# RobotControlLab/nimblephysics

Hardware: AMD Instinct MI355X
Metric: differentiable timesteps/sec (fwd+bwd), 1024-env Atlas w/ contact (higher is better)
Workload: dtype f64; 1 GPU; Atlas 33-DoF (atlas_v3_box_colliders) + ground, foot contact; worlds_per_gpu=1024, dofs=33, global_batch=1024, parallelism=independent worlds x1, launcher=single process

## Files before the change

### nimblephysics_amd/csrc/capi.cpp

```cpp
#include <hip/hip_runtime.h>

#include <cmath>
#include <cstdlib>
#include <cstdio>
#include <cstring>
#include <string>
#include <vector>

#include "model.h"
#include "pool_sizes.h"

static thread_local std::string g_err;

static int fail(int code, const std::string& msg) {
  g_err = msg;
  return code;
}

#define HIP_TRY(expr)                                                        \
  do {                                                                       \
    hipError_t _e = (expr);                                                  \
    if (_e != hipSuccess) return fail(NIMBLE_ERR_HIP, std::string(#expr) + ": " + hipGetErrorString(_e)); \
  } while (0)

// ... 171 lines not shown
    dofCount += m.ndof[b];
    if (m.jtype[b] == NIMBLE_JOINT_FREE || m.jtype[b] == NIMBLE_JOINT_BALL) {
      if (m.numFree >= 8) { delete w; return fail(NIMBLE_ERR_UNSUPPORTED, "more than 8 free / ball joints"); }
      m.freeBody[m.numFree++] = b;
    }
  }
  if (dofCount != m.n) { delete w; return fail(NIMBLE_ERR_INVALID, "dof count mismatch"); }
  {
    int k = 0;
    for (int lev = 0; lev <= m.maxDepth; lev++) {
      m.levelStart[lev] = k;
      for (int b = 0; b < m.nb; b++)
        if (m.depth[b] == lev) m.levelBodies[k++] = b;
    }
    m.levelStart[m.maxDepth + 1] = k;
    k = 0;
    for (int p = 0; p < m.nb; p++) {
      m.childStart[p] = k;
      for (int b = 0; b < m.nb; b++)
        if (m.parent[b] == p) m.childList[k++] = b;
    }
    m.childStart[m.nb] = k;
    k = 0;
    for (int lev = m.maxDepth; lev >= 1; lev--)
      for (int b = 0; b < m.nb; b++)
        if (m.depth[b] == lev && m.parent[b] >= 0) { m.accEdge[k][0] = m.parent[b]; m.accEdge[k][1] = b; k++; }
    m.numAcc = k;
  }
  for (int b = 0; b < m.nb; b++) {
    bool hasDof = false;
    for (int a = b; a >= 0; a = m.parent[a]) if (m.ndof[a] > 0) { hasDof = true; break; }
    m.reactive[b] = (d->skeleton_mobile[b] && hasDof) ? 1 : 0;
  }
  for (int i = 0; i < m.n; i++) {
    m.damping[i] = d->damping[i]; m.spring[i] = d->spring[i]; m.rest[i] = d->rest_position[i];
    m.posLo[i] = d->pos_lower[i]; m.posHi[i] = d->pos_upper[i];
    m.velLo[i] = d->vel_lower[i]; m.velHi[i] = d->vel_upper[i];
    m.forceLo[i] = d->force_lower[i]; m.forceHi[i] = d->force_upper[i];
  }
  for (int sIdx = 0; sIdx < m.ns; sIdx++) {
    m.shapeBody[sIdx] = d->shape_body[sIdx];
    m.shapeType[sIdx] = d->shape_type[sIdx];
    for (int i = 0; i < 3; i++) m.shapeSize[sIdx][i] = d->shape_size[3 * sIdx + i];
    std::memcpy(m.shapeT[sIdx], d->shape_T + 12 * sIdx, 12 * sizeof(double));
  }
  m.helperPrio = 0;
  if (const char* e = getenv("NIMBLE_AMD_HELPER_PRIO")) m.helperPrio = atoi(e) & 3;
  m.postSplit = 1;
  if (const char* e = getenv("NIMBLE_AMD_POST_SPLIT")) m.postSplit = atoi(e) != 0;
  m.pinvMfma = 1;
  if (const char* e = getenv("NIMBLE_AMD_PINV_MFMA")) m.pinvMfma = atoi(e) != 0 ? 1 : 0;
  m.bwdMFuse = 1;
  if (const char* e = getenv("NIMBLE_AMD_BWD_MFUSE")) m.bwdMFuse = atoi(e) != 0 ? 1 : 0;
  m.bwdSolve2 = 1;
  if (const char* e = getenv("NIMBLE_AMD_BWD_SOLVE2")) m.bwdSolve2 = atoi(e) != 0 ? 1 : 0;
  m.guardSites = 0;
  m.guardStride = 1;
  m.guardOffset = 0;
  if (const char* e = getenv("NIMBLE_AMD_GUARD_TEST")) {
    int sites = 0, stride = 1, offset = 0;
    if (sscanf(e, "%d:%d:%d", &sites, &stride, &offset) >= 1 && stride > 0 && offset >= 0 && offset < stride) {
      m.guardSites = sites;
      m.guardStride = stride;
      m.guardOffset = offset;
    }
  }
  m.numPairs = 0;
  m.pairChunk = 0;
  for (int i = 0; i < m.ns; i++)
    for (int j = i + 1; j < m.ns; j++) {
      int bi = m.shapeBody[i], bj = m.shapeBody[j];
      if (bi == bj) continue;
      int si = m.skel[bi], sj = m.skel[bj];
      if (!d->skeleton_mobile[bi] && !d->skeleton_mobile[bj]) continue;
      if (si == sj) continue;
      m.pairA[m.numPairs] = i;
      m.pairB[m.numPairs] = j;
      m.numPairs++;
    }
  m.pairChunk = m.numPairs < CT_PAIR_CHUNK_HOST ? m.numPairs : CT_PAIR_CHUNK_HOST;
  {
    std::vector<double> mv;
    m.hasMesh = 0;
    for (int sIdx = 0; sIdx < m.ns; sIdx++) {
      m.meshFirst[sIdx] = 0; m.meshCount[sIdx] = 0; m.meshRadius[sIdx] = 0.0;
      if (m.shapeType[sIdx] != NIMBLE_SHAPE_MESH) continue;
      if (d->mesh_vertices == nullptr || d->shape_mesh_count == nullptr || d->shape_mesh_count[sIdx] <= 0) {
        delete w;
        return fail(NIMBLE_ERR_INVALID, "mesh shape without vertices");
      }
      const int f = d->shape_mesh_first[sIdx], c = d->shape_mesh_count[sIdx];
      if (f < 0 || f + c > d->num_mesh_vertices) { delete w; return fail(NIMBLE_ERR_INVALID, "mesh vertex range"); }
      m.meshFirst[sIdx] = (int)(mv.size() / 3);
      double r2 = 0.0;
      for (int k = 0; k < c; k++) {
        const double* v = d->mesh_vertices + 3 * (size_t)(f + k);
        double q = 0.0;
        for (int i = 0; i < 3; i++) q += (v[i] * m.shapeSize[sIdx][i]) * (v[i] * m.shapeSize[sIdx][i]);
        if (q > r2) r2 = q;
        if (d->mesh_vertex_candidate != nullptr && d->mesh_vertex_candidate[f + k] == 0) continue;
        mv.insert(mv.end(), v, v + 3);
      }
      m.meshCount[sIdx] = (int)(mv.size() / 3) - m.meshFirst[sIdx];
      m.meshRadius[sIdx] = std::sqrt(r2);
      if (m.meshCount[sIdx] <= 0) {
        delete w;
// ... 43 lines not shown
    if (w->meshDev) (void)hipFree(w->meshDev);
    delete w;
    return fail(NIMBLE_ERR_UNSUPPORTED, "model too large for LDS");
  }
  w->bwd = makeLayout(m, true, bwdRows);
  w->fwdWide = w->fwd;
  w->wideLds = (size_t)w->fwd.total * sizeof(double);
  {
    const int mc = 3 * maxContacts < NIMBLE_MAX_SOLVED_LCP ? 3 * maxContacts : NIMBLE_MAX_SOLVED_LCP;
    const int wsd = 4 * mc + (mc + 1) / 2 + 3;
    int need = mc * mc + wsd + 65 * mc + 512;
    const int needL = mc * (mc | 1) + 2 * mc;
    if (needL > need) need = needL;
    const int room = (int)(160 * 1024 / sizeof(double)) - w->fwd.pool;
    const char* ev = getenv("NIMBLE_AMD_WIDE_STAGE");
    const bool on = !(ev && atoi(ev) == 0);
    if (m.numPairs > 0 && mc > 64 && on && room > 0) {
      const int cap = need < room ? need : room;
      w->fwdWide.stage = w->fwd.pool;
      w->fwdWide.stageCap = cap;
      const size_t end = (size_t)(w->fwd.pool + cap) * sizeof(double);
      if (end > w->wideLds) w->wideLds = end;
    }
    w->fwdDeferRows = w->deferRows;
    if (w->fwdWide.stageCap > 0 && fwdPoolDoublesHost(64, m.n) <= w->fwdWide.stageCap && fwdRows < w->fwdDeferRows) {
      const char* ef = getenv("NIMBLE_AMD_WIDE_POOL");
      if (!(ef && atoi(ef) == 0)) w->fwdDeferRows = fwdRows;
    }
    if (const char* e = getenv("NIMBLE_AMD_FWD_DEFER_ROWS")) {
      const int d = atoi(e);
      if (d >= 0 && d < w->fwdDeferRows && w->fwdWide.stageCap > 0) w->fwdDeferRows = d;
    }
    if (getenv("NIMBLE_AMD_VERBOSE"))
      fprintf(stderr, "nimble_amd: wide forward LDS %zu B (stage %d doubles of %d for %d rows), forward defers > %d rows\n",
              w->wideLds, w->fwdWide.stageCap, need, mc, w->fwdDeferRows);
  }
  if (getenv("NIMBLE_AMD_VERBOSE"))
    fprintf(stderr, "nimble_amd: LDS forward %d B (pool rows %d, early rows at %d), backward %d B (pool rows %d), max rows %d\n",
            w->fwd.total * 8, fwdRows, w->fwd.early, w->bwd.total * 8, bwdRows, mcap);
  const int poolRows = fwdRows < bwdRows ? fwdRows : bwdRows;
  w->poolRows = poolRows;
  w->maxRows = mcap;
  if (m.numPairs > 0) {
    int ws = 0;
    if (mcap > poolRows || mcap > w->fwdDeferRows) {
      const int a = fwdPoolDoublesHost(mcap, m.n), b = bwdPoolDoublesHost(mcap, m.n);
      ws = a > b ? a : b;
    }
    w->snapDoubles = snapWorkspaceOffsetHost(m.n) + ws;
  } else {
    w->snapDoubles = 8;
  }
  if (m.numPairs > 0 && bwdPoolDoublesHost(mcap, m.n) > w->bwd.poolCap) w->jacWsDoubles = bwdPoolDoublesHost(mcap, m.n);
  w->fwd.snDyn = w->bwd.snDyn = w->fwdWide.snDyn = w->snapDoubles;
  w->snapDoubles += dynCacheDoubles(m.n, m.nb);
  m.lay[0] = w->fwd;
  m.lay[1] = w->bwd;
  hipError_t e = hipMalloc(&w->dev, sizeof(ModelDev));
  if (e != hipSuccess) {
    if (w->meshDev) (void)hipFree(w->meshDev);
    delete w;
    return fail(NIMBLE_ERR_HIP, std::string("hipMalloc: ") + hipGetErrorString(e));
  }
  e = hipMemcpy(w->dev, &m, sizeof(ModelDev), hipMemcpyHostToDevice);
  if (e != hipSuccess) {
    (void)hipFree(w->dev);
    if (w->meshDev) (void)hipFree(w->meshDev);
    delete w;
    return fail(NIMBLE_ERR_HIP, std::string("hipMemcpy: ") + hipGetErrorString(e));
  }
  {
    std::vector<double> bi((size_t)m.nb * 10);
    for (int b = 0; b < m.nb; b++) {
      double* r = bi.data() + 10 * b;
      r[0] = m.mass[b];
      for (int i = 0; i < 3; i++) r[1 + i] = m.com[b][i];
      r[4] = m.Ic[b][0]; r[5] = m.Ic[b][4]; r[6] = m.Ic[b][8];
      r[7] = m.Ic[b][1]; r[8] = m.Ic[b][2]; r[9] = m.Ic[b][5];
    }
    e = hipMalloc(&w->inertiaDev, bi.size() * sizeof(double));
    if (e == hipSuccess) e = hipMemcpy(w->inertiaDev, bi.data(), bi.size() * sizeof(double), hipMemcpyHostToDevice);
    if (e != hipSuccess) {
      if (w->inertiaDev) (void)hipFree(w->inertiaDev);
      (void)hipFree(w->dev);
      if (w->meshDev) (void)hipFree(w->meshDev);
      delete w;
      return fail(NIMBLE_ERR_HIP, std::string("body parameters: ") + hipGetErrorString(e));
    }
  }
  *out = w;
  return NIMBLE_OK;
}

int nimble_world_destroy(nimble_world_t w) {
  if (!w) return NIMBLE_OK;
  if (w->dev) (void)hipFree(w->dev);
  if (w->inertiaDev) (void)hipFree(w->inertiaDev);
  if (w->meshDev) (void)hipFree(w->meshDev);
  delete w;
  return NIMBLE_OK;
}

int64_t nimble_snapshot_doubles(nimble_world_t w) { return w ? w->snapDoubles : -1; }
int64_t nimble_lcp_cache_doubles(nimble_world_t w) { return w ? w->cacheDoubles : -1; }
int32_t nimble_num_collision_pairs(nimble_world_t w) { return w ? w->host.numPairs : -1; }

// ... 407 lines not shown
```

### nimblephysics_amd/csrc/contact.cuh

```cuda
#pragma once
#include "model.h"
#include "spatial.cuh"
#include "pool_sizes.h"
#include "capsule.cuh"
#include "mesh.cuh"
#include "inertia.cuh"

#define CT_FACE_VERTEX 1
#define CT_VERTEX_FACE 2
#define CT_EDGE_EDGE 3
#include "stamp.cuh"

#define CM_CLAMPING (-1)
#define CM_NOT_CLAMPING (-2)


__device__ int deviceBoxBox(const double* p1, const double* R1, const double* A, const double* p2,
                            const double* R2, const double* B, double clipDepth, int b1, int b2, double* out) {
#pragma clang fp contract(off)
  const double fudge = 1.05;
  double p[3] = {p2[0] - p1[0], p2[1] - p1[1], p2[2] - p1[2]};
  double pp[3];
  for (int i = 0; i < 3; i++) pp[i] = R1[i] * p[0] + R1[3 + i] * p[1] + R1[6 + i] * p[2];
  double Rm[9], Qm[9];
// ... 2513 lines not shown
  helperWait(ct, [](int v) { return v != HS_POSTDONE; }, GW_HELPER_IDLE);
}

template <bool kWide>
__device__ void helperWave(const ModelDev& md, double* s, const Layout& L, int lane, double* g_stamp, double* hbmPool,
                           double* snap) {
  (void)g_stamp;
  s = lds<true>(s);
  double* ct = s + L.ct;
  int st = helperWait(ct, [](int v) { return v == HS_TASK || v == HS_SKIP || (!kWide && v == HS_POST); },
                      GW_HELPER_TASK);
  if (st < 0) return;
  if (!kWide && st == HS_POST) {
    helperPostShare(md, s, L, ct, snap, lane);
    return;
  }
  if (st == HS_TASK) {
    const int prio = md.helperPrio;
    if (prio == 1) __builtin_amdgcn_s_setprio(1);
    else if (prio == 2) __builtin_amdgcn_s_setprio(2);
    else if (prio == 3) __builtin_amdgcn_s_setprio(3);
    const int m = uni((int)ct[H_M]);
    const int mode = uni(helperFlags(ct)[1]);
    FwdPool P;
    if (kWide && mode == HB_WIDE) {
      carveFwd(gbl(hbmPool), m, md.n, P);
      lds_double* Ldz = (lds_double*)(s + L.pool);
      helperTask<false, 2, true>(md, ct, P, m, lane, Ldz, Ldz + dantzigLDoubles(m, true), sp<false>(P.M2), g_stamp);
    } else {
      carveFwd(s + L.pool, m, md.n, P);
      helperTask<true, 1>(md, ct, P, m, lane, sp<true>(P.M2), sp<true>(P.xh2), sp<true>(P.M2), g_stamp);
    }
  }
  __builtin_amdgcn_s_setprio(0);
  helperPost(ct, HS_DONE, lane);
  st = helperWait(ct, [](int v) { return v != HS_DONE; }, GW_HELPER_IDLE);
  if (!kWide && st == HS_POST) helperPostShare(md, s, L, ct, snap, lane);
}

__device__ __forceinline__ void helperRetire(double* s, const Layout& L, int lane) {
  double* ct = lds<true>(s) + L.ct;
  if (helperState(ct) == HS_IDLE) helperPost(ct, HS_SKIP, lane);
  helperWait(ct, [](int v) { return v == HS_DONE || v == HS_POSTDONE; }, GW_RETIRE);
  helperPost(ct, HS_IDLE, lane);
}

enum { NV_DELTA = 0, NV_NU, NV_SIGMA, NV_KAPPA, NV_MA1, NV_MARHO, NV_MA2, NV_MAPI, NV_YF, NV_W, NV_W2, NV_MU, NV_T0 };


struct BwdPool {
  double *gRows, *TAB, *NV;
  double *fc, *bc, *bounce, *u, *lam, *beta, *xq, *rho, *piv, *zeta, *r1;
  int* rowOf;
};

__device__ inline void carveBwd(double* base, int m, int n, BwdPool& P) {
  double* p = base;
  P.gRows = p; p += n * m;
  P.TAB = p; p += 12 * m;
  P.NV = p; p += NV_COLS * n;
  P.fc = p; p += m;
  P.bc = p; p += m;
  P.bounce = p; p += m;
  P.u = p; p += m;
  P.lam = p; p += m;
  P.beta = p; p += m;
  P.xq = p; p += m;
  P.rho = p; p += m;
  P.piv = p; p += m;
  P.zeta = p; p += m;
  P.r1 = p; p += m;
  P.rowOf = reinterpret_cast<int*>(p);
}

__device__ __forceinline__ unsigned long long ancestorDofMask(const ModelDev& md, unsigned long long bodies, int lane) {
  const bool in = lane < md.n && ((bodies >> md.dofBody[lane < md.n ? lane : 0]) & 1ull);
  return __ballot(in);
}

__device__ inline void bodyTwist(const ModelDev& md, const double* Sw, int b, const double* g, int ld, double* T) {
  for (int i = 0; i < 6; i++) T[i] = 0.0;
  if (b < 0) return;
  const unsigned long long a = md.anc[b];
#pragma unroll 4
  for (int r = 0; r < md.n; r++) {
    const double gr = ((a >> md.dofBody[r]) & 1ull) ? g[r * ld] : 0.0;
    for (int i = 0; i < 6; i++) T[i] = fma(Sw[6 * r + i], gr, T[i]);
  }
}

__device__ void tangentBasisGradient(const double* nrm, const double* g, double* T0, double* T1) {
  const double ez[3] = {0, 0, 1}, ex[3] = {1, 0, 0}, ey[3] = {0, 1, 0};
  const double* cr = ez;
  double t[3];
  cross3(cr, nrm, t);
  if (dot3(t, t) < 1e-12) {
    cr = ex; cross3(cr, nrm, t);
    if (dot3(t, t) < 1e-12) {
      cr = ey; cross3(cr, nrm, t);
      if (dot3(t, t) < 1e-12) { cr = ez; cross3(cr, nrm, t); }
    }
  }
  const double tn = sqrt(dot3(t, t));
  for (int i = 0; i < 3; i++) t[i] /= tn;
  double gc[3];
  cross3(cr, g, gc);
  for (int i = 0; i < 3; i++) gc[i] /= tn;
  double gt[3];
  if (fabs(tn - 1.0) > 1e-6) {
    const double dd = dot3(gc, t);
    for (int i = 0; i < 3; i++) gt[i] = gc[i] - dd * t[i];
  } else {
// ... 157 lines not shown
      rMap[q] = (int)rr[RR_MAP];
      if (rMap[q] == CM_CLAMPING) rC[q] = (int)rr[RR_CIDX];
      else if (rMap[q] >= 0) { rC[q] = (int)rows[rMap[q] * SN_ROWREC + RR_CIDX]; rE[q] = rr[RR_EVAL]; }
    }
  }
  {
    const int i = lane;
    const bool live = i < n;
    const double* nv = P.NV + (live ? i : 0) * NV_COLS;
    const double w = nv[NV_W], sg = nv[NV_SIGMA], ka = nv[NV_KAPPA], ma1 = nv[NV_MA1], mar = nv[NV_MARHO];
    const double ma2 = nv[NV_MA2], map = nv[NV_MAPI], vf = sn[SN_VF + (live ? i : 0)];
    for (int j = 0; j < m; j++) {
      const int mp = rdliR(rMap, j);
      const int c = rdliR(rC, j);
      const double e = rdlR(rE, j);
      double g = 0.0;
      if (mp == CM_CLAMPING) {
        g = P.fc[c] * w - P.beta[c] * vf - P.lam[c] * sg - P.xq[c] * ka;
        if (imp) g += P.rho[c] * ma1 + P.r1[c] * mar + P.piv[c] * ma2 + P.zeta[c] * map;
      } else if (mp >= 0) {
        double inner = P.fc[c] * w - P.xq[c] * ka;
        if (imp) inner += P.rho[c] * ma1 + P.piv[c] * ma2;
        g = e * inner;
      }
      if (live) P.gRows[j * n + i] = g;
    }
  }
  WSYNC();
  {
    auto bodyOf = [&](int t) {
      if (t >= 2 * m) return -1;
      const double* rec = sn + SN_CONTACTS + (int)rows[(t >> 1) * SN_ROWREC + RR_CONTACT] * CREC;
      return (int)rec[8 + (t & 1)];
    };
    unsigned long long anAll = 0ull;
    for (int t = lane; t < 2 * m; t += WAVE) {
      const int body = bodyOf(t);
      if (body >= 0) anAll |= md.anc[body];
    }
    unsigned lo = (unsigned)anAll, hi = (unsigned)(anAll >> 32);
    for (int o = 32; o >= 1; o >>= 1) {
      lo |= __shfl_xor(lo, o);
      hi |= __shfl_xor(hi, o);
    }
    const unsigned long long all = ((unsigned long long)uni((int)hi) << 32) | (unsigned)uni((int)lo);
    const unsigned long long dmAll = ancestorDofMask(md, all, lane);
    for (int t0 = 0; t0 < 2 * m; t0 += WAVE) {
      const int t = t0 + lane;
      const int body = bodyOf(t);
      const unsigned long long an = body >= 0 ? md.anc[body] : 0ull;
      unsigned long long dm = dmAll;
      double T[6] = {0, 0, 0, 0, 0, 0};
      const double* g = P.gRows + (t < 2 * m ? (t >> 1) : 0) * n;
      while (dm) {
        const int r = __ffsll((long long)dm) - 1;
        dm &= dm - 1ull;
        const double gr = ((an >> md.dofBody[r]) & 1ull) ? g[r] : 0.0;
        for (int i = 0; i < 6; i++) T[i] = fma(s[L.Sw + 6 * r + i], gr, T[i]);
      }
      if (t < 2 * m)
        for (int i = 0; i < 6; i++) P.TAB[(t >> 1) * 12 + (t & 1) * 6 + i] = T[i];
    }
  }
  WSYNC();
  STAMP(38);
  return imp;
}

__device__ double sphereRowTerm(const ModelDev& md, const double* s, const Layout& L, const BwdPool& P, int j,
                                const double* rec, const double* rr, const double* Z, int bk) {
  const int A = (int)rec[8], B = (int)rec[9], typ = (int)rec[7], type = typ & 15;
  const bool pa = (md.anc[A] >> bk) & 1ull, pb = (md.anc[B] >> bk) & 1ull;
  if (pa == pb) return 0.0;
  const bool sphereToBox = type == CT_SPHERE_BOX ? pa : pb;
  const int mask = (typ >> 4) & 7, shape = typ >> 8;
  const double* p = rec;
  const double* nrm = rec + 3;
  const double* c = rec + 10;
  const double wv[3] = {Z[0], Z[1], Z[2]};
  const bool rotates = sqrt(Z[0] * Z[0] + Z[1] * Z[1] + Z[2] * Z[2]) > 1e-6;
  auto gwt = [&](const double* x, double* o) {
    if (rotates) { cross3(wv, x, o); for (int i = 0; i < 3; i++) o[i] += Z[3 + i]; }
    else { for (int i = 0; i < 3; i++) o[i] = Z[3 + i]; }
  };
  auto lockProject = [&](double* x) {
    if (!mask) return;
    const double* Tw = s + L.Tw + 12 * md.shapeBody[shape];
    const double* Ts = md.shapeT[shape];
    for (int f = 0; f < 3; f++) {
      if (!((mask >> f) & 1)) continue;
      double fn[3];
      for (int r = 0; r < 3; r++) fn[r] = Tw[4 * r] * Ts[f] + Tw[4 * r + 1] * Ts[4 + f] + Tw[4 * r + 2] * Ts[8 + f];
      const double d0 = dot3(fn, x);
      for (int i = 0; i < 3; i++) x[i] -= fn[i] * d0;
    }
  };
  double sg[3], dp[3], dn[3];
  gwt(c, sg);
  double dist2 = 0.0;
  for (int i = 0; i < 3; i++) dist2 += (c[i] - p[i]) * (c[i] - p[i]);
  const double norm = sqrt(dist2);
  const double inv = norm > 1e-5 ? 1.0 / norm : 1.0;
  if (sphereToBox) {
    for (int i = 0; i < 3; i++) dp[i] = sg[i];
    lockProject(dp);
    for (int i = 0; i < 3; i++) {
      const double cpg = dp[i] * inv, spg = sg[i] * inv;
      dn[i] = type == CT_BOX_SPHERE ? cpg - spg : spg - cpg;
    }
  } else {
    double neg[3], pg[3];
// ... 355 lines not shown
  const int n = md.n, nb = md.nb;
  const double* rows = sn + SN_ROWS;
  double* omega = ws;
  double* Pc = ws + 6 * n;
  double* UV = Pc + 6 * nb;
  const int k = lane;
  const int bk = k < n ? md.dofBody[k] : 0;
  const int lam = k < n ? md.parent[bk] : -1;
  double acc = 0.0;
  unsigned long long done = 0ull;
  unsigned lo = 0u, hi = 0u;
  if (k < n) {
    if (bk < 32) lo = 1u << bk;
    else hi = 1u << (bk - 32);
  }
  for (int o = 32; o >= 1; o >>= 1) {
    lo |= __shfl_xor(lo, o);
    hi |= __shfl_xor(hi, o);
  }
  const unsigned long long dofBodies = ((unsigned long long)uni((int)hi) << 32) | (unsigned)uni((int)lo);
  int rMap[R], rA[R], rB[R], rTyp[R], rDir[R], rCon[R];
  double rp[3][R], rd[3][R], rn[3][R];
  unsigned long long liveRows[R];
#pragma unroll
  for (int q = 0; q < R; q++) {
    const int j = rowAt(q, lane);
    rMap[q] = CM_NOT_CLAMPING; rA[q] = 0; rB[q] = 0; rTyp[q] = 0; rDir[q] = 0; rCon[q] = 0;
    for (int i = 0; i < 3; i++) { rp[i][q] = 0.0; rd[i][q] = 0.0; rn[i][q] = 0.0; }
    if (j < m) {
      const double* rr = rows + j * SN_ROWREC;
      rMap[q] = (int)rr[RR_MAP];
      rDir[q] = (int)rr[RR_DIR];
      rCon[q] = (int)rr[RR_CONTACT];
      const double* rec = sn + SN_CONTACTS + rCon[q] * CREC;
      rA[q] = (int)rec[8]; rB[q] = (int)rec[9]; rTyp[q] = (int)rec[7];
      for (int i = 0; i < 3; i++) { rp[i][q] = rec[i]; rn[i][q] = rec[3 + i]; rd[i][q] = rr[RR_D + i]; }
    }
    liveRows[q] = __ballot(j < m && rMap[q] != CM_NOT_CLAMPING);
  }
  for (int j0 = 0; j0 < m; j0++) {
    if (!bitR(liveRows, j0)) continue;
    for (int side = 0; side < 2; side++) {
      const int c = side ? rdliR(rB, j0) : rdliR(rA, j0);
      if ((done >> c) & 1ull) continue;
      done |= 1ull << c;
      if (!(md.anc[c] & dofBodies)) continue;
      TACC_BEGIN(tO);
      double om[6] = {0, 0, 0, 0, 0, 0};
      unsigned long long rowsC[R];
#pragma unroll
      for (int q = 0; q < R; q++) rowsC[q] = __ballot(((liveRows[q] >> lane) & 1ull) && (rA[q] == c || rB[q] == c));
#pragma unroll
      for (int q = 0; q < R; q++)
      for (unsigned long long bits = rowsC[q]; bits; bits &= bits - 1ull) {
        const int j = 64 * q + __ffsll((long long)bits) - 1;
        const double sg = rdliR(rA, j) == c ? 1.0 : -1.0;
        double p[3], d[3];
        for (int i = 0; i < 3; i++) { p[i] = rdlR(rp[i], j); d[i] = rdlR(rd[i], j); }
        double wr[6];
        cross3(p, d, wr);
        wr[3] = d[0]; wr[4] = d[1]; wr[5] = d[2];
        if (lane < n) {
          const double gr = sg * P.gRows[j * n + lane];
#pragma unroll
          for (int i = 0; i < 6; i++) om[i] = fma(gr, wr[i], om[i]);
        }
      }
      {
        double uvl[6] = {0, 0, 0, 0, 0, 0};
#pragma unroll
        for (int q = 0; q < R; q++) {
          const int type = rTyp[q] & 15;
          const bool vertexSide = ((rowsC[q] >> lane) & 1ull) && ((type == CT_VERTEX_FACE && rA[q] == c) ||
                                                                   (type == CT_FACE_VERTEX && rB[q] == c));
          if (vertexSide) {
            const int j = rowAt(q, lane);
            double tw[3], dxt[3], pxd[3], dj[3], pj[3];
            for (int i = 0; i < 3; i++) {
              tw[i] = P.TAB[j * 12 + i] - P.TAB[j * 12 + 6 + i];
              dj[i] = rd[i][q];
              pj[i] = rp[i][q];
            }
            cross3(dj, tw, dxt);
            cross3(pj, dxt, pxd);
            for (int i = 0; i < 3; i++) { uvl[i] += dxt[i]; uvl[3 + i] += pxd[i]; }
          }
        }
        double uvs[6];
        for (int i = 0; i < 6; i++) uvs[i] = waveSum(uvl[i]);
        if (lane == 0)
          for (int i = 0; i < 6; i++) UV[i] = uvs[i];
      }
      if (lane < n)
        for (int i = 0; i < 6; i++) omega[lane * 6 + i] = om[i];
      WSYNC();
      TACC_END(82, tO);
      TACC_BEGIN(tP);
      if (lane < n) {
        double t[6];
        crf(s + L.Sw + 6 * lane, omega + 6 * lane, t);
        for (int i = 0; i < 6; i++) omega[lane * 6 + i] = t[i];
      }
      WSYNC();
      {
        unsigned long long dm = ancestorDofMask(md, md.anc[c], lane);
        if (lane < nb) {
          double pb[6] = {0, 0, 0, 0, 0, 0};
          const unsigned long long an = md.anc[lane];
          while (dm) {
            const int r = __ffsll((long long)dm) - 1;
            dm &= dm - 1ull;
            const double w = ((an >> md.dofBody[r]) & 1ull) ? 1.0 : 0.0;
#pragma unroll
            for (int i = 0; i < 6; i++) pb[i] = fma(w, omega[6 * r + i], pb[i]);
          }
          for (int i = 0; i < 6; i++) Pc[lane * 6 + i] = pb[i];
        }
      }
// ... 200 lines not shown
```

### nimblephysics_amd/csrc/model.h

```cpp
#pragma once
#include <stdint.h>

#include "../../include/nimble_amd.h"

inline int jointDofs(int jt) {
  switch (jt) {
    case NIMBLE_JOINT_WELD: return 0;
    case NIMBLE_JOINT_REVOLUTE: case NIMBLE_JOINT_PRISMATIC: return 1;
    case NIMBLE_JOINT_BALL: case NIMBLE_JOINT_TRANSLATIONAL: return 3;
    case NIMBLE_JOINT_FREE: return 6;
    default: return -1;
  }
}

#define NB_MAX NIMBLE_MAX_BODIES
#define ND_MAX NIMBLE_MAX_DOFS
#define NS_MAX NIMBLE_MAX_SHAPES

struct Layout {
  int q, v, tau, Tw, Sw, V, A, IC, F, M, rhs, x, scratch;
  int adj, Wt, w, gp, gv;
  int ct, v1, pool, poolCap, dinv;
  int snDyn;
  int cscr;
  int stage, stageCap;
  int early;
  int total;
};

struct ModelDev {
  int nb, n, ns, maxDepth;
  int numFree;
  int freeBody[8];
  double dt, g[3], clipDepth, fallbackCfm;
  int penCorr, parallelPosVel;
  int parent[NB_MAX], jtype[NB_MAX], dof0[NB_MAX], ndof[NB_MAX], depth[NB_MAX];
  int skel[NB_MAX], reactive[NB_MAX];
  unsigned long long anc[NB_MAX];
  int levelStart[NB_MAX + 1], levelBodies[NB_MAX];
  int childStart[NB_MAX + 1], childList[NB_MAX];
  int numAcc;
  int accEdge[NB_MAX][2];
  double Tpj[NB_MAX][12];
  double Tcj[NB_MAX][12];
  double TcjInv[NB_MAX][12];
  double axis[NB_MAX][3];
  double mass[NB_MAX], com[NB_MAX][3], Ic[NB_MAX][9];
  double friction[NB_MAX], restitution[NB_MAX];
  int dofBody[ND_MAX];
  double damping[ND_MAX], spring[ND_MAX], rest[ND_MAX];
  double posLo[ND_MAX], posHi[ND_MAX], velLo[ND_MAX], velHi[ND_MAX], forceLo[ND_MAX], forceHi[ND_MAX];
  int shapeBody[NS_MAX], shapeType[NS_MAX];
  double shapeSize[NS_MAX][3];
  double shapeT[NS_MAX][12];
  const double* meshVerts;
  int meshFirst[NS_MAX], meshCount[NS_MAX];
  double meshRadius[NS_MAX];
  int hasMesh;
  int helperPrio;
  int postSplit;
  int pinvMfma;
  int bwdMFuse;
  int bwdSolve2;
  int guardSites, guardStride, guardOffset;
  int maxContacts;
  int numPairs, pairChunk;
  int pairA[NS_MAX * (NS_MAX - 1) / 2], pairB[NS_MAX * (NS_MAX - 1) / 2];
  Layout lay[2];
};
```

### nimblephysics_amd/csrc/pool_sizes.h

```cpp
#pragma once
#include <hip/hip_runtime.h>

#include "../../include/nimble_amd.h"

#define CREC 13
#define EDGE_REC 12
#define PBREC (CREC + EDGE_REC)

#define CT_CONTACTS 32
#define CT_MAX_DROPPED 64
#define DROP_REC 3
#define CT_PAIR_CHUNK 16
#define CT_PAIR_CHUNK_HOST CT_PAIR_CHUNK
#define DEFER_BUCKETS 4
#define MESH_PAIR_RECS 64
#define MESH_PAIR_SCRATCH (16 * 64)
__host__ __device__ inline int ctDoubles(int maxContacts) { return CT_CONTACTS + maxContacts * CREC; }
__host__ __device__ inline int pairBufRecs(int pairChunk, bool mesh) {
  return mesh ? (MESH_PAIR_RECS > 8 * pairChunk ? MESH_PAIR_RECS : 8 * pairChunk) : 8 * pairChunk;
}
__host__ __device__ inline int collideScratchDoubles(int pairChunk, bool mesh) {
  return CT_MAX_DROPPED * DROP_REC + pairBufRecs(pairChunk, mesh) * PBREC + (mesh ? MESH_PAIR_SCRATCH : 0);
}

#define SN_NCON 0
#define SN_M 1
#define SN_NC 2
#define SN_NU 3
#define SN_CFM 4
#define SN_STATUS 5
#define SN_SC 6
#define SN_IGN 7
#define SN_IMP 8
#define SN_PIVOTS 9
#define SN_SWEEPS 10
#define SN_SOLVER_FLOPS 11
#define SN_DEFER 12
#define SN_DEFERCNT 14
#define SN_CONTACTS 16
#define SN_ROWS (SN_CONTACTS + NIMBLE_MAX_CONTACTS * CREC)
#define SN_ROWREC 12
#define SN_FC (SN_ROWS + NIMBLE_MAX_LCP * SN_ROWREC)
#define SN_VF (SN_FC + NIMBLE_MAX_LCP)
#define SN_MAXL NIMBLE_MAX_LCP
static_assert(SN_PIVOTS == NIMBLE_SNAPSHOT_PIVOTS && SN_SWEEPS == NIMBLE_SNAPSHOT_SWEEPS &&
                  SN_SOLVER_FLOPS == NIMBLE_SNAPSHOT_SOLVER_FLOPS && SN_DEFERCNT + 2 <= SN_CONTACTS,
              "include/nimble_amd.h snapshot offsets");
static_assert(SN_FC == NIMBLE_SNAPSHOT_FC && SN_NC == NIMBLE_SNAPSHOT_NUM_CLAMPING,
              "include/nimble_amd.h snapshot offsets");
__host__ __device__ inline int snAlign8(int x) { return ((x + 7) / 8) * 8; }
__host__ __device__ inline int snYf(int n) { return SN_VF + n; }
__host__ __device__ inline int snAc(int n) { return snAlign8(snYf(n) + n); }
__host__ __device__ inline int snAcubE(int n) { return snAc(n) + n * SN_MAXL; }
__host__ __device__ inline int snPT(int n) { return snAcubE(n) + n * SN_MAXL; }
__host__ __device__ inline int snQ(int n) { return snPT(n) + SN_MAXL * SN_MAXL; }
__host__ __device__ inline int snEdge(int n) { return snQ(n) + SN_MAXL * SN_MAXL; }
#ifdef NIMBLE_STAGE_TIMING
#define SN_DEBUG_TAIL 128
#else
#define SN_DEBUG_TAIL 0
#endif
__host__ __device__ inline int snStamps(int n) { return snAlign8(snEdge(n) + NIMBLE_MAX_CONTACTS * EDGE_REC); }
__host__ __device__ inline int snapWorkspaceOffset(int n) { return snStamps(n) + SN_DEBUG_TAIL; }

#define NV_COLS 16
__host__ __device__ inline int fwdPoolDoubles(int m, int n) { return n * m + 3 * m * m + 33 * m + 2 * n + 72; }
__host__ __device__ inline int bwdPoolDoubles(int m, int n) { return n * m + 24 * m + NV_COLS * n + 64; }

__host__ __device__ inline int fwdPoolRowsDoubles(int m, int n) { return n * m + 10 * m; }

#define fwdPoolDoublesHost fwdPoolDoubles
#define bwdPoolDoublesHost bwdPoolDoubles
#define snapWorkspaceOffsetHost snapWorkspaceOffset

__host__ __device__ inline int dynCacheDoubles(int n, int nb) {
  return 12 * nb + 6 * n + 6 * nb + n * (n + 1) / 2 + n + n;
}
```

### nimblephysics_amd/csrc/timestep.hip

```cpp
#include <hip/hip_runtime.h>

#include "model.h"
#include "spatial.cuh"
#include "wave.cuh"
#include "stamp.cuh"
#include "chol_wave.cuh"
#include "inertia.cuh"
#include "wrench.cuh"

#define WAVE 64

#if defined(NIMBLE_PER_WORLD_KERNELS)
#define NIMBLE_SHARED_MODEL_INSTANCES 0
#define NIMBLE_PER_WORLD_INSTANCES 1
#define NIMBLE_EXT_WRENCH_INSTANCES 0
#elif defined(NIMBLE_EXT_WRENCH_KERNELS)
#define NIMBLE_SHARED_MODEL_INSTANCES 0
#define NIMBLE_PER_WORLD_INSTANCES 0
#define NIMBLE_EXT_WRENCH_INSTANCES 1
#elif defined(__HIP__)
#define NIMBLE_SHARED_MODEL_INSTANCES 1
#define NIMBLE_PER_WORLD_INSTANCES 0
#define NIMBLE_EXT_WRENCH_INSTANCES 0
#else
// ... 609 lines not shown
  const ModelDev& md = *mdp;
  const Layout& L = md.lay[1];
  const int lane = threadIdx.x;
  const int n = md.n;
  const double dt = md.dt;
  const long long items = (long long)batch * rows;
  for (long long item = blockIdx.x; item < items; item += gridDim.x) {
    const int env = rows == 1 ? (int)item : (int)(item / rows);
    const int unitRow = rows == 1 ? -1 : (int)(item - (long long)env * rows);
    if (md.numPairs > 0) {
      const int mEnv = uni((int)snapshot[(size_t)env * snapDoubles + SN_M]);
      if ((mEnv > deferRows) != (R > 1)) continue;
    }
#ifdef NIMBLE_STAGE_TIMING
    double* g_stamp = md.numPairs > 0 ? snapshot + (size_t)env * snapDoubles + snStamps(n) : nullptr;
#endif
    STAMP(20);
    if (fcMode && (md.numPairs == 0 || unitRow >= uni((int)snapshot[(size_t)env * snapDoubles + SN_NC]))) {
      for (int i = lane; i < 2 * n; i += WAVE) gradState[(size_t)item * 2 * n + i] = 0.0;
      for (int i = lane; i < n; i += WAVE) gradForces[(size_t)item * n + i] = 0.0;
      if constexpr (kExt)
        if (gradWrench != nullptr)
          for (int i = lane; i < 6 * md.nb; i += WAVE) gradWrench[(size_t)item * 6 * md.nb + i] = 0.0;
      continue;
    }
    loadState(md, s, L, lane, state + (size_t)env * 2 * n, forces + (size_t)env * n);
    if (fcMode) {
      for (int i = lane; i < n; i += WAVE) { s[L.gp + i] = 0.0; s[L.gv + i] = 0.0; }
    } else if (unitRow < 0) {
      const double* gN = gradNext + (size_t)env * 2 * n;
      for (int i = lane; i < n; i += WAVE) {
        s[L.gp + i] = gN[i];
        s[L.gv + i] = gN[n + i];
      }
    } else {
      for (int i = lane; i < n; i += WAVE) {
        s[L.gp + i] = i == unitRow ? 1.0 : 0.0;
        s[L.gv + i] = n + i == unitRow ? 1.0 : 0.0;
      }
    }
    const double* bi = !kPW ? nullptr
                       : kExt ? bodyInertia + (size_t)env * inertiaStride
                              : bodyInertia + (size_t)env * md.nb * 10;
    double* sn = snapshot + (size_t)env * snapDoubles;
    double* hbmWs = ws != nullptr ? ws + (size_t)blockIdx.x * wsDoubles : sn + snapWorkspaceOffset(n);
    dynCacheCopy(md, s, L, sn + L.snDyn, false, lane);
    STAMP(21);
    const int nc = md.numPairs > 0 ? uni((int)sn[SN_NC]) : 0;
    const int m = md.numPairs > 0 ? uni((int)sn[SN_M]) : 0;
    double* x = s + L.x;
    double* w = s + L.w;
    BwdPool P;
    int imp = 0;
    if (nc > 0) {
      const int need = bwdPoolDoubles(m, n);
      carveBwd(need <= L.poolCap ? s + L.pool : hbmWs, m, n, P);
      imp = contactBackwardPrep<R>(md, s, L, lane, sn, P, m, nc, s + L.ct, fcMode ? unitRow : -1);
    } else {
      for (int i = lane; i < n; i += WAVE) {
        const double qi = s[L.q + i], vi = s[L.v + i];
        const double springF = md.spring[i] * (qi - md.rest[i] + dt * vi);
        const double dampF = md.damping[i] * vi;
        x[i] = dt * (s[L.tau + i] - s[L.rhs + i] - dampF - springF);
        w[i] = s[L.gv + i];
      }
      WSYNC();
      if (md.bwdSolve2) {
        double xw[2] = {lane < n ? x[lane] : 0.0, lane < n ? w[lane] : 0.0};
        cholSolveReg<2>(s + L.M, s + L.dinv, xw, n, lane);
        WSYNC();
        if (lane < n) { x[lane] = xw[0]; w[lane] = xw[1]; }
        WSYNC();
      } else {
        cholSolve(s + L.M, s + L.dinv, x, n, lane);
        cholSolve(s + L.M, s + L.dinv, w, n, lane);
      }
      for (int i = lane; i < n; i += WAVE) x[i] /= dt;
      WSYNC();
    }
    STAMP(22);
    accelerations(md, s, L, lane, x, s + L.adj);
    if constexpr (kExt) {
      adjointVectors<kPW, true>(md, s, L, lane, bi, bodyWrench + (size_t)env * md.nb * 6, wrenchFrame);
      if (gradWrench != nullptr && lane < md.nb) {
        const int b = lane;
        double Wd[6], gw[6];
        for (int i = 0; i < 6; i++) Wd[i] = dt * s[L.Wt + 6 * b + i];
        twistInWrenchFrame(Wd, wrenchFrame, s + L.Tw + 12 * b, gw);
        for (int i = 0; i < 6; i++) gradWrench[((size_t)item * md.nb + b) * 6 + i] = gw[i];
      }
    } else {
      adjointVectors<kPW>(md, s, L, lane, bi);
    }
    STAMP(23);

    double gq = 0.0, gvOut = 0.0, gt = 0.0;
    double Z[6] = {0, 0, 0, 0, 0, 0};
    const int k = lane;
    if (k < n) {
      const int b = md.dofBody[k];
      const int lam = md.parent[b];
      const double ag[6] = {0, 0, 0, md.g[0], md.g[1], md.g[2]};
      double Vl[6], ul[6];
      for (int i = 0; i < 6; i++) {
        Vl[i] = lam >= 0 ? s[L.V + 6 * lam + i] : 0.0;
        ul[i] = (lam >= 0 ? s[L.A + 6 * lam + i] : 0.0) - ag[i];
      }
      const double* Sk = s + L.Sw + 6 * k;
      if (md.jtype[b] == NIMBLE_JOINT_FREE || md.jtype[b] == NIMBLE_JOINT_BALL) {
// ... 6 lines not shown
        } else {
          double Rm[9];
          expMapRot(th, Rm);
          for (int r = 0; r < 3; r++) xi[3 + r] = Rm[(c - 3) * 3 + r];
        }
        double TwC[12];
        tmul(s + L.Tw + 12 * b, md.Tcj[b], TwC);
        adT(TwC, xi, Z);
      } else {
        for (int i = 0; i < 6; i++) Z[i] = Sk[i];
      }
      const double* a = s + L.adj + 42 * b;
      double t[6], r[6], acc6[6];
      crf(Vl, a + 6, t);
      for (int i = 0; i < 6; i++) r[i] = a[12 + i] + t[i] + a[24 + i] - a[30 + i];
      crf(Vl, r, t);
      crf(ul, a + 6, r);
      for (int i = 0; i < 6; i++) acc6[i] = -a[i] - r[i] + t[i] + a[18 + i] + a[36 + i];
      const double accQ = dot6(Z, acc6);
      double vs[6];
      for (int i = 0; i < 6; i++) vs[i] = Vl[i] + s[L.V + 6 * b + i];
      crf(vs, a + 6, t);
      for (int i = 0; i < 6; i++) acc6[i] = -t[i] - a[12 + i] - a[24 + i] + a[30 + i];
      const double accV = dot6(Sk, acc6);
      const double wk = w[k];
      gq = -dt * accQ - dt * md.spring[k] * wk;
      gvOut = s[L.gv + k] - dt * accV - dt * md.damping[k] * wk - dt * dt * md.spring[k] * wk;
      gt = dt * wk;
      if (nc > 0) gvOut -= P.NV[k * NV_COLS + NV_MU];
      if (md.jtype[b] != NIMBLE_JOINT_FREE && md.jtype[b] != NIMBLE_JOINT_BALL) {
        gq += s[L.gp + k];
        gvOut += dt * s[L.gp + k];
      }
    }
    WSYNC();
    STAMP(24);
    if (nc > 0) {
      double* buf = s + L.adj;
      TACC_BEGIN(tG);
#ifdef NIMBLE_STAGE_TIMING
      const double gterm = contactGTermsAll<R>(md, s, L, sn, P, m, Z, buf, lane, g_stamp);
#else
      const double gterm = contactGTermsAll<R>(md, s, L, sn, P, m, Z, buf, lane);
#endif
      WSYNC();
      TACC_END(80, tG);
      TACC_BEGIN(tM);
      bool mfuse = false;
      double* wI = buf + 24 * md.nb;
      const double* NVf = P.NV;
      int ldNV = NV_COLS;
      if (md.bwdMFuse) {
        const int wId = (13 * md.nb + 1) & ~1;
        const bool onChip = bwdPoolDoubles(m, n) <= L.poolCap;
        int idle = onChip ? 0 : L.poolCap;
        double* free = s + L.pool;
        if (n * (n + 1) / 2 >= wId) { mfuse = true; wI = s + L.M; }
        else if (onChip && (n + 12) * m >= wId) { mfuse = true; wI = P.gRows; }
        else if (idle >= wId) { mfuse = true; wI = free; free += wId; idle -= wId; }
        if (mfuse) {
          if (idle >= 8 * n) {
            double* stage = free;
            if (lane < n)
              for (int c = 0; c < 8; c++) stage[lane * 8 + c] = P.NV[lane * NV_COLS + c];
            NVf = stage;
            ldNV = 8;
          }
        }
      }
#ifdef NIMBLE_STAGE_TIMING
      const double mterm = mFieldsTerm<kPW>(md, s, L, NVf, ldNV, buf, wI, mfuse, lane, k, Z, -dt, (double)imp, g_stamp, bi);
#else
      const double mterm = mFieldsTerm<kPW>(md, s, L, NVf, ldNV, buf, wI, mfuse, lane, k, Z, -dt, (double)imp, bi);
#endif
      TACC_END(81, tM);
      if (k < n) {
        gq += gterm;
        gq += mterm;
      }
      WSYNC();
    }
    STAMP(25);
    if (gradMasses != nullptr) {
      if (lane < md.nb) {
        const int b = lane;
        const double* Tw = s + L.Tw + 12 * b;
        const double m = kPW ? bi[10 * b] : md.mass[b];
        const double* cb = kPW ? bi + 10 * b + 1 : md.com[b];
        double cw[3];
        for (int r = 0; r < 3; r++)
          cw[r] = Tw[r * 4] * cb[0] + Tw[r * 4 + 1] * cb[1] + Tw[r * 4 + 2] * cb[2] + Tw[r * 4 + 3];
        auto comVel = [&](const double* y, double* u) {
          double cx[3];
          cross3(cw, y, cx);
          for (int i = 0; i < 3; i++) u[i] = y[3 + i] - cx[i];
        };
        auto bodyAng = [&](const double* y, double* wb) {
          for (int i = 0; i < 3; i++) wb[i] = Tw[i] * y[0] + Tw[4 + i] * y[1] + Tw[8 + i] * y[2];
        };
        auto pairTerms = [&](const double* x, const double* y, double coef, double* out) {
          double ux[3], uy[3];
          comVel(x, ux);
          comVel(y, uy);
          out[0] += coef * (ux[0] * uy[0] + ux[1] * uy[1] + ux[2] * uy[2]);
          if (massParams < 10) return;
          for (int k = 0; k < 3; k++) {
            const double rk[3] = {Tw[k], Tw[4 + k], Tw[8 + k]};
            double a[3], c[3];
            cross3(x, rk, a);
            cross3(y, rk, c);
            out[1 + k] += coef * m * (a[0] * uy[0] + a[1] * uy[1] + a[2] * uy[2] + ux[0] * c[0] + ux[1] * c[1] + ux[2] * c[2]);
          }
          double bx[3], by[3];
          bodyAng(x, bx);
// ... 183 lines not shown
```

Measured before the change: 3.154 million timesteps/s.

## Split backward contact pool between LDS and HBM with batched off-chip row loads

Adds tiered placement for the backward contact pool. When the whole pool does not fit in LDS, only the large gRows block (or gRows plus TAB) goes to HBM workspace and the vector arrays stay on-chip. Before, everything spilled to HBM. For off-chip gRows, the TAB build loop and the omega accumulation loop batch eight row loads before the FMA work, so the global-memory latency overlaps. A host check rejects models whose tiered placement does not fit, and the NV staging path is now limited to the full-HBM tier. This adds code size and register pressure, and the gain only shows when contact rows exceed LDS capacity.

```diff
diff --git a/nimblephysics_amd/csrc/capi.cpp b/nimblephysics_amd/csrc/capi.cpp
--- a/nimblephysics_amd/csrc/capi.cpp
+++ b/nimblephysics_amd/csrc/capi.cpp
@@ -247,6 +247,8 @@
   if (const char* e = getenv("NIMBLE_AMD_PINV_MFMA")) m.pinvMfma = atoi(e) != 0 ? 1 : 0;
   m.bwdMFuse = 1;
   if (const char* e = getenv("NIMBLE_AMD_BWD_MFUSE")) m.bwdMFuse = atoi(e) != 0 ? 1 : 0;
+  m.bwdPoolSplit = 1;
+  if (const char* e = getenv("NIMBLE_AMD_BWD_POOL_SPLIT")) m.bwdPoolSplit = atoi(e) != 0 ? 1 : 0;
   m.bwdSolve2 = 1;
   if (const char* e = getenv("NIMBLE_AMD_BWD_SOLVE2")) m.bwdSolve2 = atoi(e) != 0 ? 1 : 0;
   m.guardSites = 0;
@@ -396,6 +398,18 @@
     w->snapDoubles = 8;
   }
   if (m.numPairs > 0 && bwdPoolDoublesHost(mcap, m.n) > w->bwd.poolCap) w->jacWsDoubles = bwdPoolDoublesHost(mcap, m.n);
+  if (m.numPairs > 0) {
+    const int wsSnap = w->snapDoubles - snapWorkspaceOffsetHost(m.n);
+    for (int r = 0; r <= mcap; r++) {
+      const int tier = bwdPoolTier(r, m.n, w->bwd.poolCap, m.bwdPoolSplit);
+      const int off = bwdPoolHbmDoubles(tier, r, m.n);
+      if (bwdPoolChipDoubles(tier, r, m.n) > w->bwd.poolCap || off > wsSnap || (off > 0 && off > w->jacWsDoubles)) {
+        if (w->meshDev) (void)hipFree(w->meshDev);
+        delete w;
+        return fail(NIMBLE_ERR_UNSUPPORTED, "backward pool placement does not fit for " + std::to_string(r) + " rows");
+      }
+    }
+  }
   w->fwd.snDyn = w->bwd.snDyn = w->fwdWide.snDyn = w->snapDoubles;
   w->snapDoubles += dynCacheDoubles(m.n, m.nb);
   m.lay[0] = w->fwd;
diff --git a/nimblephysics_amd/csrc/contact.cuh b/nimblephysics_amd/csrc/contact.cuh
--- a/nimblephysics_amd/csrc/contact.cuh
+++ b/nimblephysics_amd/csrc/contact.cuh
@@ -2589,12 +2589,16 @@
   double *gRows, *TAB, *NV;
   double *fc, *bc, *bounce, *u, *lam, *beta, *xq, *rho, *piv, *zeta, *r1;
   int* rowOf;
+  bool gOff;
 };
 
-__device__ inline void carveBwd(double* base, int m, int n, BwdPool& P) {
-  double* p = base;
+__device__ inline void carveBwd(double* chip, double* hbm, int tier, int m, int n, BwdPool& P) {
+  double* p = tier == BWD_TIER_CHIP ? chip : hbm;
+  P.gOff = tier != BWD_TIER_CHIP;
   P.gRows = p; p += n * m;
+  if (tier == BWD_TIER_SPLIT) p = chip;
   P.TAB = p; p += 12 * m;
+  if (tier == BWD_TIER_VEC) p = chip;
   P.NV = p; p += NV_COLS * n;
   P.fc = p; p += m;
   P.bc = p; p += m;
@@ -2858,11 +2862,32 @@
       unsigned long long dm = dmAll;
       double T[6] = {0, 0, 0, 0, 0, 0};
       const double* g = P.gRows + (t < 2 * m ? (t >> 1) : 0) * n;
+      if (!P.gOff) {
+        while (dm) {
+          const int r = __ffsll((long long)dm) - 1;
+          dm &= dm - 1ull;
+          const double gr = ((an >> md.dofBody[r]) & 1ull) ? g[r] : 0.0;
+          for (int i = 0; i < 6; i++) T[i] = fma(s[L.Sw + 6 * r + i], gr, T[i]);
+        }
+      }
       while (dm) {
-        const int r = __ffsll((long long)dm) - 1;
-        dm &= dm - 1ull;
-        const double gr = ((an >> md.dofBody[r]) & 1ull) ? g[r] : 0.0;
-        for (int i = 0; i < 6; i++) T[i] = fma(s[L.Sw + 6 * r + i], gr, T[i]);
+        int rb[8];
+        double gb[8];
+#pragma unroll
+        for (int u = 0; u < 8; u++) {
+          rb[u] = dm ? __ffsll((long long)dm) - 1 : -1;
+          dm &= dm - 1ull;
+        }
+#pragma unroll
+        for (int u = 0; u < 8; u++) {
+          const int r = rb[u] < 0 ? 0 : rb[u];
+          gb[u] = (rb[u] >= 0 && ((an >> md.dofBody[r]) & 1ull)) ? g[r] : 0.0;
+        }
+#pragma unroll
+        for (int u = 0; u < 8; u++) {
+          const int r = rb[u] < 0 ? 0 : rb[u];
+          for (int i = 0; i < 6; i++) T[i] = fma(s[L.Sw + 6 * r + i], gb[u], T[i]);
+        }
       }
       if (t < 2 * m)
         for (int i = 0; i < 6; i++) P.TAB[(t >> 1) * 12 + (t & 1) * 6 + i] = T[i];
@@ -3324,18 +3349,47 @@
       for (int q = 0; q < R; q++) rowsC[q] = __ballot(((liveRows[q] >> lane) & 1ull) && (rA[q] == c || rB[q] == c));
 #pragma unroll
       for (int q = 0; q < R; q++)
-      for (unsigned long long bits = rowsC[q]; bits; bits &= bits - 1ull) {
-        const int j = 64 * q + __ffsll((long long)bits) - 1;
-        const double sg = rdliR(rA, j) == c ? 1.0 : -1.0;
-        double p[3], d[3];
-        for (int i = 0; i < 3; i++) { p[i] = rdlR(rp[i], j); d[i] = rdlR(rd[i], j); }
-        double wr[6];
-        cross3(p, d, wr);
-        wr[3] = d[0]; wr[4] = d[1]; wr[5] = d[2];
-        if (lane < n) {
-          const double gr = sg * P.gRows[j * n + lane];
-#pragma unroll
-          for (int i = 0; i < 6; i++) om[i] = fma(gr, wr[i], om[i]);
+      for (unsigned long long bits = rowsC[q]; bits;) {
+        if (!P.gOff) {
+          const int j = 64 * q + __ffsll((long long)bits) - 1;
+          bits &= bits - 1ull;
+          const double sg = rdliR(rA, j) == c ? 1.0 : -1.0;
+          double p[3], d[3];
+          for (int i = 0; i < 3; i++) { p[i] = rdlR(rp[i], j); d[i] = rdlR(rd[i], j); }
+          double wr[6];
+          cross3(p, d, wr);
+          wr[3] = d[0]; wr[4] = d[1]; wr[5] = d[2];
+          if (lane < n) {
+            const double gr = sg * P.gRows[j * n + lane];
+#pragma unroll
+            for (int i = 0; i < 6; i++) om[i] = fma(gr, wr[i], om[i]);
+          }
+          continue;
+        }
+        int jb[8];
+        double gb[8];
+        const int jFirst = 64 * q + __ffsll((long long)bits) - 1;
+#pragma unroll
+        for (int u = 0; u < 8; u++) {
+          jb[u] = bits ? 64 * q + __ffsll((long long)bits) - 1 : -1;
+          bits &= bits - 1ull;
+        }
+#pragma unroll
+        for (int u = 0; u < 8; u++) gb[u] = (jb[u] >= 0 && lane < n) ? P.gRows[jb[u] * n + lane] : 0.0;
+#pragma unroll
+        for (int u = 0; u < 8; u++) {
+          const int j = jb[u] < 0 ? jFirst : jb[u];
+          const double sg = rdliR(rA, j) == c ? 1.0 : -1.0;
+          double p[3], d[3];
+          for (int i = 0; i < 3; i++) { p[i] = rdlR(rp[i], j); d[i] = rdlR(rd[i], j); }
+          double wr[6];
+          cross3(p, d, wr);
+          wr[3] = d[0]; wr[4] = d[1]; wr[5] = d[2];
+          if (lane < n) {
+            const double gr = sg * gb[u];
+#pragma unroll
+            for (int i = 0; i < 6; i++) om[i] = fma(gr, wr[i], om[i]);
+          }
         }
       }
       {
diff --git a/nimblephysics_amd/csrc/model.h b/nimblephysics_amd/csrc/model.h
--- a/nimblephysics_amd/csrc/model.h
+++ b/nimblephysics_amd/csrc/model.h
@@ -61,6 +61,7 @@
   int postSplit;
   int pinvMfma;
   int bwdMFuse;
+  int bwdPoolSplit;
   int bwdSolve2;
   int guardSites, guardStride, guardOffset;
   int maxContacts;
diff --git a/nimblephysics_amd/csrc/pool_sizes.h b/nimblephysics_amd/csrc/pool_sizes.h
--- a/nimblephysics_amd/csrc/pool_sizes.h
+++ b/nimblephysics_amd/csrc/pool_sizes.h
@@ -67,6 +67,23 @@
 __host__ __device__ inline int fwdPoolDoubles(int m, int n) { return n * m + 3 * m * m + 33 * m + 2 * n + 72; }
 __host__ __device__ inline int bwdPoolDoubles(int m, int n) { return n * m + 24 * m + NV_COLS * n + 64; }
 
+enum { BWD_TIER_CHIP = 1, BWD_TIER_SPLIT = 2, BWD_TIER_VEC = 3, BWD_TIER_HBM = 4 };
+__host__ __device__ inline int bwdPoolHbmDoubles(int tier, int m, int n) {
+  return tier == BWD_TIER_CHIP    ? 0
+         : tier == BWD_TIER_SPLIT ? n * m
+         : tier == BWD_TIER_VEC   ? (n + 12) * m
+                                  : bwdPoolDoubles(m, n);
+}
+__host__ __device__ inline int bwdPoolChipDoubles(int tier, int m, int n) {
+  return bwdPoolDoubles(m, n) - bwdPoolHbmDoubles(tier, m, n);
+}
+__host__ __device__ inline int bwdPoolTier(int m, int n, int poolCap, int split) {
+  if (bwdPoolDoubles(m, n) <= poolCap) return BWD_TIER_CHIP;
+  if (split && bwdPoolChipDoubles(BWD_TIER_SPLIT, m, n) <= poolCap) return BWD_TIER_SPLIT;
+  if (split && bwdPoolChipDoubles(BWD_TIER_VEC, m, n) <= poolCap) return BWD_TIER_VEC;
+  return BWD_TIER_HBM;
+}
+
 __host__ __device__ inline int fwdPoolRowsDoubles(int m, int n) { return n * m + 10 * m; }
 
 #define fwdPoolDoublesHost fwdPoolDoubles
diff --git a/nimblephysics_amd/csrc/timestep.hip b/nimblephysics_amd/csrc/timestep.hip
--- a/nimblephysics_amd/csrc/timestep.hip
+++ b/nimblephysics_amd/csrc/timestep.hip
@@ -685,9 +685,9 @@
     double* w = s + L.w;
     BwdPool P;
     int imp = 0;
+    const int tier = bwdPoolTier(m, n, L.poolCap, md.bwdPoolSplit);
     if (nc > 0) {
-      const int need = bwdPoolDoubles(m, n);
-      carveBwd(need <= L.poolCap ? s + L.pool : hbmWs, m, n, P);
+      carveBwd(s + L.pool, hbmWs, tier, m, n, P);
       imp = contactBackwardPrep<R>(md, s, L, lane, sn, P, m, nc, s + L.ct, fcMode ? unitRow : -1);
     } else {
       for (int i = lane; i < n; i += WAVE) {
@@ -800,14 +800,14 @@
       int ldNV = NV_COLS;
       if (md.bwdMFuse) {
         const int wId = (13 * md.nb + 1) & ~1;
-        const bool onChip = bwdPoolDoubles(m, n) <= L.poolCap;
-        int idle = onChip ? 0 : L.poolCap;
-        double* free = s + L.pool;
+        const int used = tier == BWD_TIER_CHIP ? L.poolCap : bwdPoolChipDoubles(tier, m, n);
+        int idle = L.poolCap - used;
+        double* free = s + L.pool + used;
         if (n * (n + 1) / 2 >= wId) { mfuse = true; wI = s + L.M; }
-        else if (onChip && (n + 12) * m >= wId) { mfuse = true; wI = P.gRows; }
+        else if (tier == BWD_TIER_CHIP && (n + 12) * m >= wId) { mfuse = true; wI = P.gRows; }
         else if (idle >= wId) { mfuse = true; wI = free; free += wId; idle -= wId; }
         if (mfuse) {
-          if (idle >= 8 * n) {
+          if (tier == BWD_TIER_HBM && idle >= 8 * n) {
             double* stage = free;
             if (lane < n)
               for (int c = 0; c < 8; c++) stage[lane * 8 + c] = P.NV[lane * NV_COLS + c];
```

Measured after the change: 3.188 million timesteps/s, median of 6. 1.01x the previous value.
